# nanoporetech/scrappie

Hardware: AMD Instinct MI355X
Metric: raw samples/sec, rgrgr_r94 4k-sample reads (higher is better)
Workload: dtype f32 (3xf16 split products, 22-bit operands, fp32 accumulate)

## Files before the change

scrappie_amd/csrc/sh_eng_launch.inc:

```

struct MetaPtrs { ShMeta md; const long long *seq_off, *hp_off, *bases_off; ShGruLanes lanes, lanes1; ShGruPairs pairs, pairs2; const ShGruSegD *vseg, *vlseg; const int *vloff; ShDwellArgs dw; };

#define SH_DWELL_PER_ENTRY 10
static long long bases_reservation(long long per_entry, long long nentry) { return (per_entry * nentry + 16 + 15) & ~15ll; }
extern "C" size_t scrappie_hip_dwell_capacity(size_t nentry) { return (size_t)bases_reservation(SH_DWELL_PER_ENTRY, (long long)nentry); }

static int build_group(scrappie_hip_engine *e, Slot &sl, Model *m, const uint64_t *offsets, const uint32_t *lengths,
                       size_t n, bool hp_on, MetaPtrs &mp, const DwellJob *dw = nullptr, const PostJob *pj = nullptr) {
    LaunchGroup &lg = sl.lg;
    lg.valid = false;
    lg.n = n; lg.hp_on = hp_on;
    lg.dw = DwellJob();
    if (dw && dw->on) {
        if (m->arch != 3 || dw->off.size() != n || dw->num.size() != n || dw->host.size() != n) return set_err("build_group: %zu reads, dwells of %zu", n, dw->off.size());
        lg.dw = *dw;
    }
    lg.post = PostJob(); lg.npost = 0;
    if (pj && pj->on) {
        if (m->arch != 1 || pj->dst.size() != n) return set_err("build_group: base probabilities of %zu reads for a group of %zu (flip-flop models only)", pj->dst.size(), n);
        lg.post = *pj;
    }
    lg.ntile = (n + 15) / 16; lg.npad = lg.ntile * 16;
    const int st = m->stride;
    std::vector<int> T(n);
// ... 254 lines not shown
#ifdef SH_EXPERIMENTS
            if constexpr (nu() == 6)
                if (stamp) return launch_k<k_gru_lanes<6, true>>(lgrid, dim3(768), lds, s, xaff, out, resid, sW, sW2, md, backward, lanes, st.dev(4096 * 16 * 8));
#endif
            return launch_k<k_gru_lanes<nu(), false>>(lgrid, dim3(128 * nu()), lds, s, xaff, out, resid, sW, sW2, md, backward, lanes, (unsigned long long *)nullptr);
            })) return set_err("unsupported GRU size %d (need 32, 64 or 96 here)", S);
        if (stamp && NU == 6)
            st.dump_on(7, s, (size_t)nwg * 12 * 8, [&](const unsigned long long *h) {
                for (size_t g : {(size_t)nwg / 2}) for (int w = 0; w < 12; w++) {
                    const unsigned long long *d = &h[(g * 12 + w) * 8];
                    fprintf(stderr, "gru lanes stamp wg %zu wave %2d: phase1 %.0f bar %.0f phase2 %.0f bar %.0f cycles/step (%llu steps)\n",
                            g, w, d[0] / (double)d[4], d[1] / (double)d[4], d[2] / (double)d[4], d[3] / (double)d[4], d[4]);
                }
            });
        return rc;
    }
    if (tun().gru_debug >= 0) backward |= tun().gru_debug << 8;
    static StampBuf st1;
    unsigned long long *dbgbuf = tun().gru_stamp ? st1.dev(4096 * 8 * 8) : nullptr;
    if (dbgbuf)
        st1.dump_on(8, s, ntile * NU * 8, [&](const unsigned long long *h) {
            { unsigned long long first_end = ~0ull, mn = ~0ull, mx = 0; size_t late = 0;
              for (size_t tl = 0; tl < ntile; tl++) { first_end = std::min(first_end, h[tl * NU * 8 + 7]); mn = std::min(mn, h[tl * NU * 8 + 6]); mx = std::max(mx, h[tl * NU * 8 + 7]); }
              for (size_t tl = 0; tl < ntile; tl++) if (h[tl * NU * 8 + 6] >= first_end) late++;
              fprintf(stderr, "residency: %zu tiles, %zu started after the first one finished; span %.1f us\n", ntile, late, (mx - mn) / 100.0); }
            for (size_t tl : {size_t(0)}) for (int w = 0; w < 1; w++) {
                const unsigned long long *d = &h[(tl * NU + w) * 8];
                fprintf(stderr, "stamp tile %zu wave %d: rgemm %.0f zgemm+valu %.0f bar1 %.0f gemm2+valu %.0f bar2 %.0f (cycles/step)\n", tl, w, d[0] / (double)d[5], d[1] / (double)d[5], d[2] / (double)d[5], d[3] / (double)d[5], d[4] / (double)d[5]);
            }
        });
    if (pick_int<2, 4, 6, 8>(NU, rc, [&](auto nu) { return launch_k<k_gru<nu()>>(dim3((unsigned)ntile), dim3(64 * nu()), 0, s, xaff, out, resid, sW, sW2, md, backward, dbgbuf); })) return rc;
    return set_err("unsupported GRU size %d (need 32, 64, 96 or 128)", S);
}

#ifndef SH_FFL_NB
#define SH_FFL_NB 3
#endif
#ifndef SH_FFL_NTH
#define SH_FFL_NTH 512
#endif
static int ff_mtp(int KQ, int mtiles) {
    const size_t per_mt = ((size_t)KQ * 256 + 256) * 4;
    int mt_fit = (int)((156 * 1024) / per_mt);
    mt_fit -= mt_fit % SH_SUM_GROUP;
    return std::min(mt_fit, (mtiles + SH_SUM_GROUP - 1) / SH_SUM_GROUP * SH_SUM_GROUP);
}

template <int KQ>
static int launch_ff_lds_k(hipStream_t s, const float *in, float *E, float *sums, const unsigned *wf, const float *bf,
                           long long ncb, int mtiles, int NS, float in_div, float out_div, int ncu) {
    constexpr int NB = SH_FFL_NB, NTH = SH_FFL_NTH;
    const int mtp = ff_mtp(KQ, mtiles);
    const size_t lds = (size_t)mtp * ((size_t)KQ * 256 + 256) * 4 + 16;
    long long gx = std::min<long long>((ncb + (NTH / 64) * NB - 1) / ((NTH / 64) * NB), ncu);
    if (gx < 1) gx = 1;
    const bool dv = out_div != 1.0f;
    const bool stamp = tun().ff_stamp && !dv;
    static StampBuf st;
    unsigned long long *dbg = stamp ? st.dev(16 * 8) : nullptr;
    if (pick_bool([&](auto d) { return launch_k<k_ff_lds<KQ, NB, NTH, d()>>(dim3((unsigned)gx), dim3(NTH), lds, s, in, E, sums, wf, bf, ncb, mtiles, mtp, NS, in_div, out_div, dbg); }, dv))
        return -1;
    if (stamp)
        st.dump_on(0, s, NTH / 64 * 8, [](const unsigned long long *h) {
            for (int w = 0; w < NTH / 64; w++)
                fprintf(stderr, "ff stamp wave %d: fill %llu  B-load %llu  tiles %llu  sums %llu cycles; %llu m-tiles -> %.0f cycles per m-tile\n", w, h[w * 8], h[w * 8 + 1], h[w * 8 + 2], h[w * 8 + 3], h[w * 8 + 4], (double)h[w * 8 + 2] / (double)h[w * 8 + 4]);
        });
    return 0;
}

static int launch_ff(hipStream_t s, int S, const float *in, float *E, float *sums, const unsigned *wf, const float *bf,
                     long long ncb, int mtiles, int NS, float in_div, float out_div, int ncu) {
    int rc = 0;
    if (ncb >= 8192 && !tun().ff_reg &&
        pick_int<2, 4, 6>(S / 16, rc, [&](auto kq) { return launch_ff_lds_k<kq()>(s, in, E, sums, wf, bf, ncb, mtiles, NS, in_div, out_div, ncu); })) return rc;
    constexpr int NB = SH_FF_NB;
    const int mtp = ff_mtp(S / 16, mtiles);
    const long long gx = (ncb + 4 * NB - 1) / (4 * NB);
    dim3 grid((unsigned)std::max<long long>(gx, 1));
    if (pick_int<2, 4, 6, 8>(S / 16, rc, [&](auto kq) {
            constexpr int KQ = kq();
            return pick_bool([&](auto dv) { return launch_k<k_ff_exp<KQ, NB, dv()>>(grid, dim3(256), 0, s, in, E, sums, wf, bf, ncb, mtiles, mtp, NS, in_div, out_div); },
                             out_div != 1.0f);
        })) return rc;
    return set_err("unsupported size %d", S);
}

static bool gru_proj_ok(int K, int S) { return K == S && S % 32 == 0 && S / 16 <= 6; }

static bool conv_edge_words(const ShConvGeom &g, int N, int T, int out[4]) {
    out[0] = out[1] = out[2] = out[3] = 0;
    if (T <= 0) return true;
    unsigned irr = 0;
    bool ok = true;
    for (int t = std::max(g.c0, T - 64); t < T; t++) {
        const int kk = (t - g.c0) / g.nstepC, ii = (t - g.c0) - kk * g.nstepC;
        if (!((kk + 1) * g.nstepX <= N - g.shiftX - ii * g.st)) {
            const int j = T - 1 - t;
            if (j >= 32) ok = false; else irr |= 1u << j;
        }
    }
    const int maxCol = (N - g.shiftX) / g.nstepX;
    const int rem = (N - g.shiftX) % g.nstepX;
    const int colR = g.c0 + g.nstepC * (maxCol - 1) + rem / g.st + 1;
    const int startR = g.st - (g.padL + N - g.WL) % g.st - 1;
    out[0] = (int)irr; out[1] = colR + startR / g.st; out[2] = startR; out[3] = N;
    return ok;
}

extern "C" int scrappie_hip_conv_edge_words(int WL, int st, int F, int N, int out[4]) {
    if (WL < 1 || st < 1 || N < 1 || !out) return -1;
    return conv_edge_words(conv_geom(WL, st, F), N, (N + st - 1) / st, out) ? 1 : 0;
}

#ifdef SH_EXPERIMENTS
static int launch_gru_conv(hipStream_t s, int kst, int act, float *out, const unsigned *iW, const float *ib, const unsigned *sW,
                           const unsigned *sW2, const ShMeta &md, int backward, const ShGruLanes &lanes1, int nwg1,
                           const ShGruLanes &lanes2, int nwg2, bool two, const ShConvFuse &cf) {
    const ShGruLanes &lanes = two ? lanes2 : lanes1;
    const int nwg = two ? nwg2 : nwg1;
    if (nwg <= 0) return 0;
    HIPCHK(hipMemsetAsync(lanes.flag, 0, (size_t)lanes.ntile * 4, s));
    const size_t lds = (two ? 2 : 1) * ((size_t)4 * 3 * 2 * 64 * 4 + (size_t)2 * 3 * 6 * 256) * 4;
    dim3 grid((unsigned)nwg);
    if (tun().proj_stamp && two && kst == 3 && !act) {
        static StampBuf st;
        if (launch_k<k_gru_conv_stamp<2, 3, 0>>(grid, dim3(768), lds, s, out, iW, ib, sW, sW2, md, backward, lanes, cf, st.dev(1024 * 12 * 16))) return -1;
        st.dump_on(3, s, (size_t)nwg * 12 * 16, [&](const unsigned long long *h) {
            for (int w = 0; w < 12; w++) {
                const unsigned long long *d = &h[((size_t)(nwg / 2) * 12 + w) * 16];
                fprintf(stderr, "conv-layer stamp wave %2d (%s): A %.0f bar %.0f B %.0f bar %.0f cycles per double step (%llu steps); chunk+fetch part of B (projection) / reads+MFMA issue (recurrence) %.0f\n", w,
                        w < 6 ? "recurrence" : "projection", d[0] / (double)d[4], d[1] / (double)d[4], d[2] / (double)d[4], d[3] / (double)d[4], d[4], d[5] / (double)d[4]);
            }
        });
        return 0;
    }
    return pick_bool([&](auto t2, auto k3, auto ac) {
        return launch_k<k_gru_conv<t2() ? 2 : 1, k3() ? 3 : 5, ac() ? 1 : 0>>(grid, dim3(768), lds, s, out, iW, ib, sW, sW2, md, backward, lanes, cf);
    }, two, kst == 3, act != 0);
}
#endif
static int launch_gru_proj(hipStream_t s, int S, const float *in, float *out, const float *resid, const unsigned *iW, const float *ib,
                           const unsigned *sW, const unsigned *sW2, const ShMeta &md, int backward, const ShGruLanes &lanes1, int nwg1,
                           const ShGruLanes &lanes2, int nwg2, bool two) {
    const ShGruLanes &lanes = two ? lanes2 : lanes1;
    const int nwg = two ? nwg2 : nwg1;
    if (nwg <= 0) return 0;
    HIPCHK(hipMemsetAsync(lanes.flag, 0, (size_t)lanes.ntile * 4, s));
    const int NU = S / 16;
    size_t lds = (two ? 2 : 1) * ((size_t)4 * (NU / 2) * 2 * 64 * 4 + (size_t)2 * 3 * NU * 256) * 4;
    if (resid && SH_RESID_LDS && lds + (size_t)(two ? 2 : 1) * 3 * NU * 256 * 4 <= 160 * 1024) lds += (size_t)(two ? 2 : 1) * 3 * NU * 256 * 4;
    dim3 grid((unsigned)nwg);
    unsigned long long *const no_dbg = nullptr;
    int rc = 0;
#ifdef SH_EXPERIMENTS
    static const bool mx_on = [] { const char *v = getenv("SH_GRU_MX"); return v && atoi(v) != 0; }();
    if (mx_on && NU == 6 && two) {
        static const bool mx_stamp = getenv("SH_MX_STAMP") != nullptr;
        if (mx_stamp && !resid) {
            static StampBuf st;
            if (launch_k<k_gru_mx<false, true>>(grid, dim3(1024), lds, s, in, out, resid, iW, ib, sW, sW2, md, backward, lanes, st.dev((size_t)1024 * 16 * 10))) return -1;
            st.dump_on(7, s, (size_t)nwg * 16 * 10, [&](const unsigned long long *hb) {
                for (int w = 0; w < 16; w++) {
                    const unsigned long long *d = &hb[((size_t)(nwg / 2) * 16 + w) * 10];
                    const double n = (double)std::max<unsigned long long>(d[8], 1);
                    fprintf(stderr, "mx stamp wave %2d (%s): P1 %.0f +bar %.0f | P2 %.0f +bar %.0f | P3 %.0f +bar %.0f | P4 %.0f +bar %.0f cycles per double step (%llu steps)\n", w,
                            w < 6 ? "recurrence " : w < 12 ? "projection " : "elementwise", d[0] / n, d[1] / n, d[2] / n, d[3] / n, d[4] / n, d[5] / n, d[6] / n, d[7] / n, d[8]);
                }
            });
            return 0;
        }
        if (pick_bool([&](auto rs) { return launch_k<k_gru_mx<rs()>>(grid, dim3(1024), lds, s, in, out, resid, iW, ib, sW, sW2, md, backward, lanes, no_dbg); }, resid != nullptr))
            return -1;
        HIPCHK(hipGetLastError());
        return 0;
    }
    const bool stamp = tun().proj_stamp && NU == 6 && two && !resid;
    const bool free_run = SH_GRU_FREE_DEFAULT ? !tun().gru_barrier : tun().gru_free;
    if (free_run) {
        const size_t flds = (two ? 2 : 1) * ((size_t)4 * (NU / 2) * 2 * 64 * 4 + (size_t)3 * 3 * NU * 256) * 4 + 64;
        if (stamp) {
            static StampBuf st;
            if (launch_k<k_gru_free<6, 2, false, true>>(grid, dim3(768), flds, s, in, out, resid, iW, ib, sW, sW2, md, backward, lanes, st.dev(1024 * 12 * 16))) return -1;
            st.dump_on(7, s, (size_t)nwg * 12 * 16, [&](const unsigned long long *h) {
                for (int w = 0; w < 12; w++) {
                    const unsigned long long *d = &h[((size_t)(nwg / 2) * 12 + w) * 16];
                    if (w < 6) fprintf(stderr, "free stamp wave %2d (recurrence): work %.0f, waiting for gate inputs %.0f, for r*h of all waves %.0f, for h of all waves %.0f cycles per double step (%llu steps)\n",
                                       w, d[0] / (double)d[4], d[1] / (double)d[4], d[2] / (double)d[4], d[3] / (double)d[4], d[4]);
                    else fprintf(stderr, "free stamp wave %2d (projection): work %.0f, waiting for the column's pieces %.0f, for a free ring slot %.0f cycles per double step (%llu steps)\n",
                                 w, d[0] / (double)d[4], d[1] / (double)d[4], d[2] / (double)d[4], d[4]);
                }
            });
            return 0;
        }
        if (pick_int<2, 4, 6>(NU, rc, [&](auto nu) {
                constexpr int N = nu();
                return pick_bool([&](auto t2, auto rs) {
                    return launch_k<k_gru_free<N, t2() ? 2 : 1, rs(), false>>(grid, dim3(128 * N), flds, s, in, out, resid, iW, ib, sW, sW2, md, backward, lanes, no_dbg);
                }, two, resid != nullptr);
            })) return rc;
        return set_err("unsupported GRU size %d (need 32, 64 or 96 here)", S);
    }
    if (stamp) {
        static StampBuf st;
        if (launch_k<k_gru_proj<6, 2, false, true>>(grid, dim3(768), lds, s, in, out, resid, iW, ib, sW, sW2, md, backward, lanes, st.dev(1024 * 12 * 16))) return -1;
        st.dump_on(7, s, (size_t)nwg * 12 * 16, [&](const unsigned long long *h) {
            for (int w = 0; w < 12; w++) {
                const unsigned long long *d = &h[((size_t)(nwg / 2) * 12 + w) * 16];
                fprintf(stderr, "proj stamp wave %2d (%s): A %.0f bar %.0f B %.0f bar %.0f cycles per double step (%llu steps)", w, w < 6 ? "recurrence" : "projection",
                        d[0] / (double)d[4], d[1] / (double)d[4], d[2] / (double)d[4], d[3] / (double)d[4], d[4]);
                if (w < 6) fprintf(stderr, "; inside B: reads+MFMA issue %.0f, logistic z %.0f, tanh+blend %.0f, store+bookkeeping %.0f, cut+publish %.0f",
                                   d[5] / (double)d[4], d[6] / (double)d[4], d[7] / (double)d[4], d[8] / (double)d[4], d[9] / (double)d[4]);
                fprintf(stderr, "\n");
            }
        });
        return 0;
    }
#endif
    if (pick_int<2, 4, 6>(NU, rc, [&](auto nu) {
            constexpr int N = nu();
            return pick_bool([&](auto t2) {
                constexpr int NT = t2() ? 2 : 1;
                if (resid) return launch_k<k_gru_proj_res<N, NT>>(grid, dim3(128 * N), lds, s, in, out, resid, iW, ib, sW, sW2, md, backward, lanes);
                return launch_k<k_gru_proj<N, NT, false>>(grid, dim3(128 * N), lds, s, in, out, resid, iW, ib, sW, sW2, md, backward, lanes, no_dbg);
            }, two);
        })) return rc;
    return set_err("unsupported GRU size %d (need 32, 64 or 96 here)", S);
}

#ifdef SH_EXPERIMENTS
#ifndef SH_GRU32_DEFAULT
#define SH_GRU32_DEFAULT 0
#endif
static int use_gru32(const scrappie_hip_engine *e) {
    if (e->dbg_gru32 >= 0) return e->dbg_gru32;
    if (SH_GRU32_DEFAULT ? tun().gru16 : !tun().gru32) return 0;
    const char *v = getenv("SH_GRU32");
    return (v && atoi(v) == 2) ? 2 : (SH_GRU32_DEFAULT ? SH_GRU32_DEFAULT : 1);
}
static const char *const g32_role[8] = {"R0 chain", "R1 chain", "R2 chain", "C cand-proj", "G0 z/r", "G1 z/r", "G2 z/r", "L loader"};
static int launch_gru_proj32x2(hipStream_t s, const float *in, float *out, bool resid, const unsigned *iW, const float *ib, const unsigned *sW,
                               const unsigned *sW2, const ShMeta &md, int backward, const ShGruPairs &pairs, int nwg, size_t ntile) {
    if (nwg <= 0) return 0;
    HIPCHK(hipMemsetAsync(pairs.flag, 0, ntile * 4, s));
    const size_t lds = (size_t)SH_G32X2_LDS_WORDS * 4;
    dim3 grid((unsigned)nwg);
    if (tun().gru32_stamp && !resid) {
        static StampBuf st;
        if (launch_k<k_gru_proj32x2<false, true>>(grid, dim3(512), lds, s, in, out, iW, ib, sW, sW2, md, backward, pairs, st.dev(1024 * 8 * 16))) return -1;
        st.dump_on(7, s, (size_t)nwg * 8 * 16, [&](const unsigned long long *h) {
            for (int w = 0; w < 8; w++) {
                const unsigned long long *d = &h[((size_t)(nwg / 2) * 8 + w) * 16];
                fprintf(stderr, "gru32x2 stamp wave %d (%s): work %.0f bar %.0f cycles per interval (%llu intervals = one tile-step of 32 reads each)\n", w, g32_role[w],
                        d[0] / (double)d[4], d[1] / (double)d[4], d[4]);
            }
        });
        return 0;
    }
    return pick_bool([&](auto rs) { return launch_k<k_gru_proj32x2<rs(), false>>(grid, dim3(512), lds, s, in, out, iW, ib, sW, sW2, md, backward, pairs, (unsigned long long *)nullptr); }, resid);
}
static int launch_gru_proj32(hipStream_t s, const float *in, float *out, bool resid, const unsigned *iW, const float *ib, const unsigned *sW,
                             const unsigned *sW2, const ShMeta &md, int backward, const ShGruPairs &pairs, int nwg, size_t ntile) {
    if (nwg <= 0) return 0;
    HIPCHK(hipMemsetAsync(pairs.flag, 0, ntile * 4, s));
    const size_t lds = (size_t)SH_G32_LDS_WORDS * 4;
    dim3 grid((unsigned)nwg);
    if (tun().gru32_stamp && !resid) {
        static StampBuf st;
        if (launch_k<k_gru_proj32<false, true>>(grid, dim3(512), lds, s, in, out, iW, ib, sW, sW2, md, backward, pairs, st.dev(1024 * 8 * 16))) return -1;
        st.dump_on(7, s, (size_t)nwg * 8 * 16, [&](const unsigned long long *h) {
            for (int w = 0; w < 8; w++) {
                const unsigned long long *d = &h[((size_t)(nwg / 2) * 8 + w) * 16];
                fprintf(stderr, "gru32 stamp wave %d (%s): A %.0f bar %.0f B %.0f bar %.0f cycles per step (%llu steps)", w, g32_role[w],
                        d[0] / (double)d[4], d[1] / (double)d[4], d[2] / (double)d[4], d[3] / (double)d[4], d[4]);
                if (w < 3) fprintf(stderr, "; A: reads+r products %.0f, logistic*h %.0f, cut+write %.0f; B: reads+candidate products %.0f, z/tanh/blend %.0f, store %.0f, cut+write %.0f",
                                   d[5] / (double)d[4], d[6] / (double)d[4], d[7] / (double)d[4], d[8] / (double)d[4], d[9] / (double)d[4], d[10] / (double)d[4], d[11] / (double)d[4]);
                fprintf(stderr, "\n");
            }
        });
        return 0;
    }
    return pick_bool([&](auto rs) { return launch_k<k_gru_proj32<rs(), false>>(grid, dim3(512), lds, s, in, out, iW, ib, sW, sW2, md, backward, pairs, (unsigned long long *)nullptr); }, resid);
}

#endif
static int launch_lstm(hipStream_t s, int S, const float *xaff, float *out, const unsigned *sW, const float *pf,
                       const ShMeta &md, int backward, const ShGruLanes &lanes, int nwg) {
    if (nwg <= 0) return 0;
    HIPCHK(hipMemsetAsync(lanes.flag, 0, (size_t)lanes.ntile * 4, s));
    int rc = 0;
    if (pick_int<2, 4, 6>(S / 16, rc, [&](auto nu) { return launch_k<k_lstm_lanes<nu()>>(dim3((unsigned)nwg), dim3(128 * nu()), 0, s, xaff, out, sW, pf, md, backward, lanes); })) return rc;
    return set_err("unsupported LSTM size %d (need 32, 64 or 96)", S);
}

static int launch_lstm_proj(hipStream_t s, int S, int I, const float *in, float *out, const unsigned *iW, const float *ib,
                            const unsigned *sW, const float *pf, const ShMeta &md, int backward, const ShGruLanes &lanes, int nwg) {
    if (nwg <= 0) return 0;
    HIPCHK(hipMemsetAsync(lanes.flag, 0, (size_t)lanes.ntile * 4, s));
    const int NU = S / 16;
    const size_t lds = ((size_t)4 * (NU / 2) * 2 * 64 * 4 + (size_t)2 * 4 * NU * 256 + (size_t)3 * NU * 256) * 4;
    if (I != S && I != 16) return set_err("unsupported LSTM input width %d", I);
    int rc = 0;
    if (pick_int<2, 4, 6>(NU, rc, [&](auto nu) {
            constexpr int N = nu();
            return pick_bool([&](auto wide) { return launch_k<k_lstm_proj<N, wide() ? N : 1>>(dim3((unsigned)nwg), dim3(128 * N), lds, s, in, out, iW, ib, sW, pf, md, backward, lanes); },
                             I == S);
        })) return rc;
    return set_err("unsupported LSTM size %d (need 32, 64 or 96)", S);
}

static size_t viterbi_lds_bytes(int NH) {
    const int nskip = NH / 16, nslip = std::max(NH / 64, 1);
    return (size_t)NH * 16 * 4 * 2 + (size_t)nskip * 16 * 8 + (size_t)nslip * 16 * 8 + 2 * 16 * 16 * 8;
}

static int launch_viterbi(hipStream_t s, int NH, const ShVitArgs &a, const ShMeta &md, size_t nwg) {
    const size_t lds = viterbi_lds_bytes(NH);
    if (nwg == 0) return 0;
    const bool fin = a.sums != nullptr, slip = a.use_slip != 0, skip0 = a.skip_pen == 0.0f;
    if (fin && !a.want_log) return set_err("decode: exp-value input implies log output");
    const auto go = [&](auto nth, auto ppt) {
        constexpr int NTH = nth(), PPT = ppt();
        return pick_bool([&](auto fi, auto sl, auto sk) { return launch_k<k_viterbi<NTH, PPT, fi(), sl(), sk()>>(dim3((unsigned)nwg), dim3(NTH), lds, s, a, md); },
                         fin, slip, skip0);
    };
    switch (NH) {
    case 64: return go(int_c<256>(), int_c<1>());
    case 256: return go(int_c<256>(), int_c<4>());
    case 1024:
#ifdef SH_EXPERIMENTS
        if (getenv("SH_VIT_1024")) return go(int_c<1024>(), int_c<4>());
#endif
        return go(int_c<512>(), int_c<8>());
    default: return set_err("unsupported transducer state count %d (need 4^3, 4^4 or 4^5 k-mers)", NH);
    }
}

static int launch_ff_viterbi(hipStream_t s, const ShFfArgs &f, const ShVitArgs &a, const ShMeta &md, size_t nwg, bool single) {
    const size_t lds = (size_t)SH_FV_LDS_FLOATS * 4;
    if (nwg == 0) return 0;
    dim3 grid((unsigned)nwg);
    const bool slip = a.use_slip != 0, skip0 = a.skip_pen == 0.0f, dv = f.out_div != 1.0f || f.in_div != 1.0f;
    if (!a.use_slip && !single) {
        const size_t ldt = (size_t)SH_FVT_LDS_FLOATS * 4;
        static const bool keep_clamp = getenv("SH_FVT_KEEP_CLAMP") != nullptr;
        const bool nc = f.no_clamp && !dv && !keep_clamp;
        return pick_bool([&](auto sk, auto d, auto n) {
            if constexpr (d() && n()) return -1;
            else return launch_k<k_ff_viterbi_teams<sk(), d(), n()>>(grid, dim3(SH_FVT_NTH), ldt, s, f, a, md);
        }, skip0, dv, nc);
    }
    return pick_bool([&](auto sl, auto sk, auto d) { return launch_k<k_ff_viterbi<sl(), sk(), d()>>(grid, dim3(512), lds, s, f, a, md); }, slip, skip0, dv);
}
```

scrappie_amd/csrc/sh_gru.h:

```cpp
#ifndef SH_GRU_H
#define SH_GRU_H

template <int NU>
__global__ __launch_bounds__(64 * NU) void k_gru(const float *__restrict__ xaff, float *__restrict__ out,
                                                 const float *__restrict__ resid,
                                                 const float *__restrict__ sWfrag ,
                                                 const float *__restrict__ sW2frag ,
                                                 ShMeta md, int backward, unsigned long long *dbgbuf) {
    constexpr int KR = NU * 4;
    const int dbg = backward >> 8;
    backward &= 1;
    __shared__ __attribute__((aligned(16))) float lds[2 * NU * 256];
    float *lds_h = lds, *lds_rh = lds + NU * 256;
    const int lane = threadIdx.x & 63, u = threadIdx.x >> 6;
    const int tile = blockIdx.x;
    const int Tt = md.tile_T[tile];
    const long long boff = md.tile_boff[tile];
    const int myT = md.rT[tile * 16 + (lane & 15)];

    float wz[KR], wr[KR], wh[KR];
#pragma unroll
    for (int r = 0; r < KR; r++) {
        wz[r] = sWfrag[((long long)u * KR + r) * 64 + lane];
        wr[r] = sWfrag[((long long)(NU + u) * KR + r) * 64 + lane];
// ... 325 lines not shown
    auto fetch_next = [&](int i) {
        n_ok = i < sge;
        if (n_ok) {
            const ShGruSegD sg = L.seg[i];
            n_tile = __builtin_amdgcn_readfirstlane(sg.tile);
            n_s0 = __builtin_amdgcn_readfirstlane(sg.s0);
            n_s1 = __builtin_amdgcn_readfirstlane(sg.s1);
            n_Tt = __builtin_amdgcn_readfirstlane(md.tile_T[n_tile]);
            n_boff = __builtin_amdgcn_readfirstlane((int)md.tile_boff[n_tile]);
            n_myT = md.rT[n_tile * 16 + (lane & 15)];
        }
    };
    auto advance = [&]() { tile = n_tile; s = n_s0; s1 = n_s1; Tt = n_Tt; boff = n_boff; myT = n_myT; };
    f32x4 h = {0.f, 0.f, 0.f, 0.f};
    auto take_over = [&]() {
        h = (f32x4){0.f, 0.f, 0.f, 0.f};
        if (s > 0) {
            if (!sh_wait_flag(L.flag + tile, (unsigned)NU, L.flag + L.ntile) && lane == 0)
                __hip_atomic_store(L.flag + L.ntile, 1u, __ATOMIC_RELAXED, __HIP_MEMORY_SCOPE_AGENT);
            __builtin_amdgcn_fence(__ATOMIC_ACQUIRE, "agent");
            const float *hs = L.hstate + ((long long)tile * NU + u) * 256 + lane * 4;
#pragma unroll
            for (int k = 0; k < 4; k++) h[k] = __hip_atomic_load(hs + k, __ATOMIC_RELAXED, __HIP_MEMORY_SCOPE_AGENT);
        }
    };
    f32x4 xz = h, xr = h, xh = h;
    auto xload = [&](long long col) {
        const float *p = xaff + col * xstride + lane * 4;
        xz = *(const f32x4 *)(p + u * 256);
        xr = *(const f32x4 *)(p + (NU + u) * 256);
        xh = *(const f32x4 *)(p + (2 * NU + u) * 256);
    };
    if (my_it > 0) {
        fetch_next(sgi);
        advance();
        fetch_next(++sgi);
        take_over();
        publish(lds_h, h);
        xload(boff + (backward ? Tt - 1 - s : s));
    }
    __syncthreads();

    int it = 0;
    for (; it < my_it; it++) {
        f32x4 ar = xr * SH_OSCALE, az = xz * SH_OSCALE, ah = xh * SH_OSCALE;
        const int t = backward ? Tt - 1 - s : s;
        {
            long long ncol = boff + t;
            if (s + 1 < s1) ncol = boff + (backward ? t - 1 : t + 1);
            else if (n_ok) ncol = n_boff + (backward ? n_Tt - 1 - n_s0 : n_s0);
            xload(ncol);
        }
        {
            ShSplit hp[KS];
#pragma unroll
            for (int ks = 0; ks < KS; ks++) hp[ks] = pieces(lds_h, ks);
            split_dot2<KS>(wr, wz, hp, ar, az);
        }
        publish(lds_rh, d_logistic4_acc(ar) * h);
        const f32x4 z = d_logistic4_acc(az);
        lds_barrier();
        {
            ShSplit rp[KS];
#pragma unroll
            for (int ks = 0; ks < KS; ks++) rp[ks] = pieces(lds_rh, ks);
            ah = split_dot<KS>(wh, rp, ah);
        }
        const bool active = t < myT;
        {
            const f32x4 hbar = d_tanh4_acc(ah);
            const f32x4 hn = z * h + (1.0f - z) * hbar;
#pragma unroll
            for (int k = 0; k < 4; k++) h[k] = active ? hn[k] : 0.0f;
        }
        f32x4 o = h;
        const long long oidx = ((long long)(boff + t) * NU + u) * 256 + lane * 4;
        if (resid) o += *(const f32x4 *)(resid + oidx);
        *(f32x4 *)(out + oidx) = o;
        s++;
        if (s == s1) {
            if (s1 < Tt) {
                float *hs = L.hstate + ((long long)tile * NU + u) * 256 + lane * 4;
#pragma unroll
                for (int k = 0; k < 4; k++) __hip_atomic_store(hs + k, h[k], __ATOMIC_RELAXED, __HIP_MEMORY_SCOPE_AGENT);
                __builtin_amdgcn_fence(__ATOMIC_RELEASE, "agent");
                if (lane == 0) __hip_atomic_fetch_add(L.flag + tile, 1u, __ATOMIC_RELEASE, __HIP_MEMORY_SCOPE_AGENT);
            }
            if (n_ok) {
                advance();
                fetch_next(++sgi);
                take_over();
            }
        }
        publish(lds_h, h);
        lds_barrier();
    }
    for (; it < nit; it++) { lds_barrier(); lds_barrier(); }
}

struct ShLaneCursor {
    int sgi, sge;
    int tile, s, s1, Tt, boff;
    bool ok;
};

#ifndef SH_REC45_PRIO
#define SH_REC45_PRIO 0
#endif
#ifndef SH_REC_PRIO
#define SH_REC_PRIO 0
#endif
#ifndef SH_PDELAY_A
#define SH_PDELAY_A 0
#endif
#ifndef SH_PDELAY_B
#define SH_PDELAY_B 0
#endif
#ifndef SH_PROJ_PRIO
#define SH_PROJ_PRIO 0
#endif
#ifndef SH_RFIRST
#define SH_RFIRST 1
#endif
#ifndef SH_PROJ_VALU_FIRST
#define SH_PROJ_VALU_FIRST 1
#endif
#ifndef SH_PROJ_INPLACE
#define SH_PROJ_INPLACE 1
#endif
#ifndef SH_ABL
#define SH_ABL 0
#endif
__device__ __forceinline__ f32x4 abl_logistic4(f32x4 a) { return (SH_ABL & 1) ? a * (0.25f * SH_OINV) + 0.5f : d_logistic4_acc(a); }
__device__ __forceinline__ f32x4 abl_tanh4(f32x4 a) { return (SH_ABL & 1) ? a * (0.5f * SH_OINV) : d_tanh4_acc(a); }

#ifndef SH_GRU_VGPR_HALF
#define SH_GRU_VGPR_HALF 72
#endif
#ifndef SH_FUSE_ABL
#define SH_FUSE_ABL 0
#endif
struct ShConvFuse {
    const float *sig;
    const float *W;
    const float *bias;
    const int *edge;
    unsigned *bad;
    ShConvGeom g;
};

#ifndef SH_RESID_LDS
#define SH_RESID_LDS 1
#endif
template <int NU, int NT, bool RESID, bool STAMP, int KST, int ACT>
__device__ __forceinline__ void gru_proj_body(const float *__restrict__ in, float *__restrict__ out,
                                              const float *__restrict__ resid,
                                              const unsigned *__restrict__ iWp, const float *__restrict__ ibfrag,
                                              const unsigned *__restrict__ sWp, const unsigned *__restrict__ sW2p,
                                              const ShMeta &md, int backward, const ShGruLanes &L,
                                              unsigned long long *dbg, const ShConvFuse &cf) {
    constexpr bool CONV = KST > 0;
    static_assert(NU % 2 == 0, "k steps of 32 units");
    constexpr int KS = NU / 2;
    constexpr int PBUF = KS * 2 * 64 * 4;
    constexpr int XBUF = 3 * NU * 256;
    constexpr int TBUF = 4 * PBUF + 2 * XBUF;
    constexpr int RBUF = NU * 256;
    constexpr bool RLDS = RESID && !CONV && SH_RESID_LDS && (NT * (TBUF + 3 * RBUF) * 4 <= 160 * 1024);
    unsigned long long pa = 0, pb = 0, pc = 0, pd = 0, pt0 = 0, pt1;
    unsigned long long q1 = 0, q2 = 0, q3 = 0, q4 = 0, q5 = 0, qt0 = 0, qt1;
#define QSTAMP(acc) do { if (STAMP) { qt1 = __builtin_readcyclecounter(); acc += qt1 - qt0; qt0 = qt1; } } while (0)
#define PSTAMP(acc) do { if (STAMP) { pt1 = __builtin_readcyclecounter(); acc += pt1 - pt0; pt0 = pt1; } } while (0)
#define PDUMP() do { if (STAMP && dbg && lane == 0) { unsigned long long *d_ = dbg + ((long long)blockIdx.x * 2 * NU + wave) * 16; d_[0] = pa; d_[1] = pb; d_[2] = pc; d_[3] = pd; d_[4] = nit; d_[5] = q1; d_[6] = q2; d_[7] = q3; d_[8] = q4; d_[9] = q5; } } while (0)
    extern __shared__ __attribute__((aligned(16))) unsigned ldsw[];
    const int lane = threadIdx.x & 63;
    const unsigned lofs = (unsigned)lane * 4u;
    typedef __attribute__((address_space(1))) float *gf32;
    typedef __attribute__((address_space(1))) f32x4 *gf32x4;
    auto gload = [&](const float *base) { gf32 b = (gf32)base; asm volatile("" : "+s"(b)); return *(gf32x4)(b + lofs); };
    auto gstore = [&](float *base, f32x4 v) { gf32 b = (gf32)base; asm volatile("" : "+s"(b)); *(gf32x4)(b + lofs) = v; };
    const int wave = __builtin_amdgcn_readfirstlane(threadIdx.x >> 6);
    const bool rec = wave < NU;
    const int u = rec ? wave : wave - NU;

    ShSplit w0[KS], w1[KS], w2[KS];
    {
        const unsigned *f0 = rec ? sWp + (long long)u * KS * 512 : iWp + (long long)u * KS * 512;
        const unsigned *f1 = rec ? sWp + (long long)(NU + u) * KS * 512 : iWp + (long long)(NU + u) * KS * 512;
        const unsigned *f2 = rec ? sW2p + (long long)u * KS * 512 : iWp + (long long)(2 * NU + u) * KS * 512;
#pragma unroll
        for (int ks = 0; ks < KS; ks++) {
            w0[ks] = load_pieces(f0 + ks * 512, lane);
            w1[ks] = load_pieces(f1 + ks * 512, lane);
            w2[ks] = load_pieces(f2 + ks * 512, lane);
        }
#pragma unroll
        for (int ks = 0; ks < KS; ks++)
            asm volatile("" : "+v"(w0[ks].p1), "+v"(w0[ks].p2), "+v"(w1[ks].p1), "+v"(w1[ks].p2), "+v"(w2[ks].p1), "+v"(w2[ks].p2));
    }
    const int wofs = (((u >> 1) * 2) * 64 + lane) * 4 + (u & 1) * 2;
    auto publish = [&](unsigned *buf, f32x4 v) {
        unsigned a1, a2, b1, b2;
        if (SH_ABL & 4) { a1 = __float_as_uint(v[0]); a2 = __float_as_uint(v[1]); b1 = __float_as_uint(v[2]); b2 = __float_as_uint(v[3]); }
        else { split_pair(v[0], v[1], a1, a2); split_pair(v[2], v[3], b1, b2); }
        *(uint2 *)(buf + wofs) = make_uint2(a1, b1);
        *(uint2 *)(buf + wofs + 256) = make_uint2(a2, b2);
    };
    auto pieces = [&](const unsigned *buf, int ks) { return load_pieces(buf + ks * 512, lane); };
    auto lds_h = [&](int tl) { return ldsw + tl * TBUF; };
    auto lds_rh = [&](int tl) { return ldsw + tl * TBUF + PBUF; };
    auto lds_in = [&](int tl, int par) { return ldsw + tl * TBUF + (2 + par) * PBUF; };
    auto lds_x = [&](int tl, int par) { return (float *)(ldsw + tl * TBUF + 4 * PBUF + par * XBUF); };
    auto lds_raw = [&](int tl, int slot) { return (float *)(ldsw + NT * TBUF + (tl * 3 + slot) * RBUF) + (u * 64 + lane) * 4; };

    ShLaneCursor c[NT] = {};
    int my_it[NT], nit = 0;
#pragma unroll
    for (int tl = 0; tl < NT; tl++) {
        const int ln = blockIdx.x * NT + tl;
        c[tl].sgi = __builtin_amdgcn_readfirstlane(L.lane_off[ln]);
        c[tl].sge = __builtin_amdgcn_readfirstlane(L.lane_off[ln + 1]);
        int n = 0;
        for (int i = c[tl].sgi; i < c[tl].sge; i++) n += L.seg[i].s1 - L.seg[i].s0;
        my_it[tl] = __builtin_amdgcn_readfirstlane(n);
        nit = max(nit, my_it[tl]);
    }
    if (nit == 0) return;
    auto enter = [&](ShLaneCursor &cc) {
        cc.ok = cc.sgi < cc.sge;
        if (cc.ok) {
            const ShGruSegD sg = L.seg[cc.sgi];
            cc.tile = __builtin_amdgcn_readfirstlane(sg.tile);
            cc.s = __builtin_amdgcn_readfirstlane(sg.s0);
            cc.s1 = __builtin_amdgcn_readfirstlane(sg.s1);
            cc.Tt = __builtin_amdgcn_readfirstlane(md.tile_T[cc.tile]);
            cc.boff = __builtin_amdgcn_readfirstlane((int)md.tile_boff[cc.tile]);
        }
    };
    auto column = [&](const ShLaneCursor &cc) { return (long long)cc.boff + (backward ? cc.Tt - 1 - cc.s : cc.s); };

    if (!rec) {
        if (SH_PROJ_PRIO) __builtin_amdgcn_s_setprio(SH_PROJ_PRIO);
        f32x4 bz = *(const f32x4 *)(ibfrag + (u * 64 + lane) * 4);
        f32x4 br = *(const f32x4 *)(ibfrag + ((NU + u) * 64 + lane) * 4);
        asm volatile("" : "+v"(bz), "+v"(br));
        f32x4 bh = *(const f32x4 *)(ibfrag + ((2 * NU + u) * 64 + lane) * 4);
        asm volatile("" : "+v"(bh));
        int e_irr[NT], e_pw[NT], e_N[NT], e_T[NT];
        unsigned e_soff[NT];
        float ca[CONV ? KST : 1];
        f32x4 cb = {0.f, 0.f, 0.f, 0.f};
        auto read_consts = [&](int tl) {
            if (CONV && c[tl].ok) {
                const int rd = c[tl].tile * 16 + (lane & 15);
                const int4 ev = ((const int4 *)cf.edge)[rd];
                e_irr[tl] = ev.x; e_pw[tl] = ev.y * 16 + ev.z; e_N[tl] = ev.w;
                e_T[tl] = md.rT[rd];
                e_soff[tl] = (unsigned)md.sig_off[rd];
            }
        };
        if (CONV) {
#pragma unroll
            for (int ks = 0; ks < (CONV ? KST : 1); ks++)
                ca[ks] = (4 * ks + (lane >> 4) < cf.g.WL) ? cf.W[(4 * ks + (lane >> 4)) * cf.g.F + 16 * u + (lane & 15)] : 0.0f;
            cb = *(const f32x4 *)(cf.bias + 16 * u + 4 * (lane >> 4));
#pragma unroll
            for (int tl = 0; tl < NT; tl++) { e_irr[tl] = 0; e_pw[tl] = 0; e_N[tl] = 0; e_T[tl] = 0; e_soff[tl] = 0u; }
        }
        struct XQ { f32x4 v; float xs[CONV ? KST : 1]; int meta; int tile; };
        auto fetch = [&](ShLaneCursor &cc, int tl) {
            XQ x;
            x.meta = 0; x.tile = 0;
            if constexpr (!CONV) {
                const long long col = cc.ok ? column(cc) : 0;
                x.v = gload(in + (col * NU + u) * 256);
            } else {
                const int tb = cc.ok ? (backward ? cc.Tt - 1 - cc.s : cc.s) : 0;
                const bool live = cc.ok && tb < e_T[tl];
                const int j = e_T[tl] - 1 - tb;
                const bool regular = live && !(j < 32 && ((e_irr[tl] >> (j & 31)) & 1));
                const int base = tb * cf.g.st - cf.g.padL + (lane >> 4);
                typedef __attribute__((address_space(1))) float *gsf;
                gsf sb = (gsf)cf.sig; asm volatile("" : "+s"(sb));
                int okbits = 0;
#pragma unroll
                for (int ks = 0; ks < KST; ks++) {
                    const int idx = base + 4 * ks;
                    const bool ok = regular && 4 * ks + (lane >> 4) < cf.g.WL && idx >= 0 && idx < e_N[tl];
                    x.xs[ks] = (SH_FUSE_ABL & 1) ? (float)idx : *(sb + (e_soff[tl] + (unsigned)(ok ? idx : 0)));
                    okbits |= ok ? (256 << ks) : 0;
                }
                const int jw = tb - (e_pw[tl] >> 4);
                const int wp = (e_pw[tl] & 15) + jw * cf.g.st;
                x.meta = (live ? ((jw >= 0 && wp < cf.g.padR) ? wp + 2 : 1) : 0) | okbits;
                x.tile = cc.tile;
            }
            if (cc.ok) {
                cc.s++;
                if (cc.s == cc.s1) { cc.sgi++; enter(cc); read_consts(tl); }
            }
            return x;
        };
        auto chunk_of = [&](const XQ &x) {
            if constexpr (!CONV) return x.v;
            else {
                f32x4 acc = cb;
#pragma unroll
                for (int ks = 0; ks < KST; ks++) { if (SH_FUSE_ABL & 2) acc[0] += ca[ks] * x.xs[ks]; else acc = mfma4(ca[ks], ((x.meta >> (8 + ks)) & 1) ? x.xs[ks] : 0.0f, acc); }
                const int rd = x.tile * 16 + (lane & 15);
                const int colcode = x.meta & 255;
                if (!(SH_FUSE_ABL & 4) && colcode >= 2) {
                    const int N = md.rN[rd], w = colcode - 2;
                    const float *xp = cf.sig + md.sig_off[rd] + (N - cf.g.WL + 1 + w);
                    const int f0 = 16 * u + 4 * (lane >> 4);
                    for (int tap = 0; tap < cf.g.WL - w - 1; tap++) {
                        const f32x4 wv = *(const f32x4 *)(cf.W + tap * cf.g.F + f0);
                        acc += wv * xp[tap];
                    }
                }
                if (colcode == 0) acc = f32x4{0.f, 0.f, 0.f, 0.f};
                else if (!(SH_FUSE_ABL & 8)) {
                    bool out_of_range = false;
#pragma unroll
                    for (int r = 0; r < 4; r++) {
                        const float v = ACT ? d_tanh(acc[r]) : d_elu(acc[r]);
                        out_of_range |= !(__builtin_fabsf(v) < SH_ACT_LIMIT) | !(__builtin_fabsf(acc[r]) <= 3.0e38f);
                        acc[r] = (v == v) ? __builtin_amdgcn_fmed3f(v, -SH_ACT_LIMIT, SH_ACT_LIMIT) : 0.0f;
                    }
                    if (out_of_range && cf.bad) cf.bad[rd] = 1u;
                }
                return acc;
            }
        };
        XQ xq1[NT], xq2[NT];
        auto project_h = [&](const unsigned *ibuf, float *xdst) {
            ShSplit ip[KS];
#pragma unroll
            for (int ks = 0; ks < KS; ks++) ip[ks] = pieces(ibuf, ks);
            const f32x4 dst = (SH_ABL & 8) ? bh : split_dot<KS>(w2, ip, bh);
            *(f32x4 *)(xdst + ((2 * NU + u) * 64 + lane) * 4) = dst;
            if ((SH_ABL & 16) && !(u == 2 || u == 3)) {
                const f32x4 extra = split_dot<KS>(w0, ip, bh);
                asm volatile("" :: "v"(extra));
            }
        };
        auto project_zr = [&](const unsigned *ibuf, float *xdst) {
            f32x4 cz = bz, cr = br;
            if (!(SH_ABL & 8) && !((SH_ABL & 16) && (u == 2 || u == 3))) {
                ShSplit ip[KS];
#pragma unroll
                for (int ks = 0; ks < KS; ks++) ip[ks] = pieces(ibuf, ks);
                split_dot2<KS>(w0, w1, ip, cz, cr);
            }
            *(f32x4 *)(xdst + (u * 64 + lane) * 4) = cz;
            *(f32x4 *)(xdst + ((NU + u) * 64 + lane) * 4) = cr;
        };
#pragma unroll
        for (int tl = 0; tl < NT; tl++) {
            enter(c[tl]);
            read_consts(tl);
            const XQ xin = fetch(c[tl], tl);
            xq1[tl] = fetch(c[tl], tl); xq2[tl] = fetch(c[tl], tl);
            publish(lds_in(tl, 0), chunk_of(xin));
            if constexpr (RLDS) *(f32x4 *)lds_raw(tl, 0) = chunk_of(xin);
        }
        lds_barrier();
#pragma unroll
        for (int tl = 0; tl < NT; tl++) {
            project_h(lds_in(tl, 0), lds_x(tl, 0));
            project_zr(lds_in(tl, 0), lds_x(tl, 0));
            publish(lds_in(tl, 1), chunk_of(xq1[tl]));
            if constexpr (RLDS) *(f32x4 *)lds_raw(tl, 1) = chunk_of(xq1[tl]);
            xq1[tl] = xq2[tl];
            xq2[tl] = fetch(c[tl], tl);
        }
        lds_barrier();
        if (STAMP) pt0 = __builtin_readcyclecounter();
        int wslot = 2;
        if constexpr (CONV || SH_PROJ_INPLACE) {
            auto step = [&](int it, const int par, XQ (&e)[NT]) {
                const int np = par ^ 1;
#pragma unroll
                for (int tl = 0; tl < NT; tl++) project_h(lds_in(tl, np), lds_x(tl, np));
                PSTAMP(pa);
                lds_barrier();
                PSTAMP(pb);
#pragma unroll
                for (int tl = 0; tl < NT; tl++) {
                    publish(lds_in(tl, par), chunk_of(e[tl]));
                    if constexpr (RLDS) *(f32x4 *)lds_raw(tl, wslot) = chunk_of(e[tl]);
                    e[tl] = fetch(c[tl], tl);
                }
                if constexpr (RLDS) wslot = wslot == 2 ? 0 : wslot + 1;
                __builtin_amdgcn_sched_barrier(0);
                if (STAMP) { qt1 = __builtin_readcyclecounter(); q1 += qt1 - pt0; }
#pragma unroll
                for (int tl = 0; tl < NT; tl++) project_zr(lds_in(tl, np), lds_x(tl, np));
                PSTAMP(pc);
                lds_barrier();
                PSTAMP(pd);
            };
            for (int it = 0; it < nit; it += 2) {
                step(it, 0, xq1);
                if (it + 1 < nit) step(it + 1, 1, xq2);
            }
        } else
        for (int it = 0; it < nit; it++) {
            const int np = (it + 1) & 1;
            if (SH_PDELAY_A) __builtin_amdgcn_s_sleep(SH_PDELAY_A);
#pragma unroll
            for (int tl = 0; tl < NT; tl++) project_h(lds_in(tl, np), lds_x(tl, np));
            PSTAMP(pa);
            lds_barrier();
            PSTAMP(pb);
            if (SH_PROJ_VALU_FIRST) {
#pragma unroll
                for (int tl = 0; tl < NT; tl++) {
                    publish(lds_in(tl, it & 1), chunk_of(xq1[tl]));
                    if constexpr (RLDS) *(f32x4 *)lds_raw(tl, wslot) = chunk_of(xq1[tl]);
                    xq1[tl] = xq2[tl];
                    xq2[tl] = fetch(c[tl], tl);
                }
                __builtin_amdgcn_sched_barrier(0);
            }
            if (SH_PDELAY_B) __builtin_amdgcn_s_sleep(SH_PDELAY_B);
#pragma unroll
            for (int tl = 0; tl < NT; tl++) project_zr(lds_in(tl, np), lds_x(tl, np));
            if (!SH_PROJ_VALU_FIRST) {
#pragma unroll
                for (int tl = 0; tl < NT; tl++) {
                    publish(lds_in(tl, it & 1), chunk_of(xq1[tl]));
                    if constexpr (RLDS) *(f32x4 *)lds_raw(tl, wslot) = chunk_of(xq1[tl]);
                    xq1[tl] = xq2[tl];
                    xq2[tl] = fetch(c[tl], tl);
                }
            }
            if constexpr (RLDS) wslot = wslot == 2 ? 0 : wslot + 1;
            PSTAMP(pc);
            lds_barrier();
            PSTAMP(pd);
        }
        PDUMP();
        return;
    }

    if (SH_REC_PRIO) __builtin_amdgcn_s_setprio(SH_REC_PRIO);
    if (SH_REC45_PRIO && NU == 6 && wave >= 4) __builtin_amdgcn_s_setprio(SH_REC45_PRIO);
    static_assert(NT <= 2, "two block counts per register");
    unsigned myT2 = 0;
    f32x4 h[NT];
    auto take_over = [&](int tl) {
        h[tl] = (f32x4){0.f, 0.f, 0.f, 0.f};
        int mt = 0;
        if (c[tl].ok) mt = md.rT[c[tl].tile * 16 + (lane & 15)];
        if (NT == 1) myT2 = (unsigned)mt;
        else myT2 = tl ? ((myT2 & 0xffffu) | ((unsigned)mt << 16)) : ((myT2 & 0xffff0000u) | ((unsigned)mt & 0xffffu));
        if (!c[tl].ok) return;
        if (c[tl].s > 0) {
            if (!sh_wait_flag(L.flag + c[tl].tile, (unsigned)NU, L.flag + L.ntile) && lane == 0)
                __hip_atomic_store(L.flag + L.ntile, 1u, __ATOMIC_RELAXED, __HIP_MEMORY_SCOPE_AGENT);
            __builtin_amdgcn_fence(__ATOMIC_ACQUIRE, "agent");
            const float *hs = L.hstate + ((long long)c[tl].tile * NU + u) * 256 + lane * 4;
#pragma unroll
            for (int k = 0; k < 4; k++) h[tl][k] = __hip_atomic_load(hs + k, __ATOMIC_RELAXED, __HIP_MEMORY_SCOPE_AGENT);
        }
        asm volatile("" : "+v"(myT2), "+v"(h[tl][0]), "+v"(h[tl][1]), "+v"(h[tl][2]), "+v"(h[tl][3]));
    };
    long long oix[NT];
    const long long dstep = backward ? -(long long)(NU * 256) : (long long)(NU * 256);
    auto cur_off = [&](int tl) {
        const long long v = c[tl].ok ? (column(c[tl]) * NU + u) * 256 : (long long)(u * 256);
        const unsigned lo = __builtin_amdgcn_readfirstlane((unsigned)v), hi = __builtin_amdgcn_readfirstlane((unsigned)(v >> 32));
        return (long long)(((unsigned long long)hi << 32) | lo);
    };
#pragma unroll
    for (int tl = 0; tl < NT; tl++) {
        enter(c[tl]);
        take_over(tl);
        oix[tl] = cur_off(tl);
        publish(lds_h(tl), h[tl]);
    }
    lds_barrier();
    lds_barrier();
    if (STAMP) pt0 = __builtin_readcyclecounter();
    f32x4 rs[NT];
    auto resid_fetch = [&](int tl) {
        rs[tl] = gload(resid + oix[tl]);
    };
    if (RESID && !RLDS) {
#pragma unroll
        for (int tl = 0; tl < NT; tl++) resid_fetch(tl);
    }
    int rslot = 0;
    for (int it = 0; it < nit; it++) {
        const int par = it & 1;
        f32x4 cr[NT], cz[NT];
        f32x4 z[NT];
        if (SH_RFIRST) {
            ShSplit hp[NT][KS];
#pragma unroll
            for (int tl = 0; tl < NT; tl++) {
                const float *xs = lds_x(tl, par);
                cz[tl] = *(const f32x4 *)(xs + (u * 64 + lane) * 4);
                cr[tl] = *(const f32x4 *)(xs + ((NU + u) * 64 + lane) * 4);
#pragma unroll
                for (int ks = 0; ks < KS; ks++) hp[tl][ks] = pieces(lds_h(tl), ks);
                cr[tl] = split_dot<KS>(w1, hp[tl], cr[tl]);
            }
#pragma unroll
            for (int tl = 0; tl < NT; tl++) cz[tl] = split_dot<KS>(w0, hp[tl], cz[tl]);
#pragma unroll
            for (int tl = 0; tl < NT; tl++) publish(lds_rh(tl), abl_logistic4(cr[tl]) * h[tl]);
        } else {
#pragma unroll
        for (int tl = 0; tl < NT; tl++) {
            const float *xs = lds_x(tl, par);
            cz[tl] = *(const f32x4 *)(xs + (u * 64 + lane) * 4);
            cr[tl] = *(const f32x4 *)(xs + ((NU + u) * 64 + lane) * 4);
            ShSplit hp[KS];
#pragma unroll
            for (int ks = 0; ks < KS; ks++) hp[ks] = pieces(lds_h(tl), ks);
            split_dot2<KS>(w1, w0, hp, cr[tl], cz[tl]);
        }
#pragma unroll
        for (int tl = 0; tl < NT; tl++) {
            publish(lds_rh(tl), abl_logistic4(cr[tl]) * h[tl]);
            z[tl] = abl_logistic4(cz[tl]);
        }
        }
        PSTAMP(pa);
        lds_barrier();
        PSTAMP(pb);
        if (STAMP) qt0 = __builtin_readcyclecounter();
        f32x4 ch[NT];
#pragma unroll
        for (int tl = 0; tl < NT; tl++) {
            ShSplit rp[KS];
#pragma unroll
            for (int ks = 0; ks < KS; ks++) rp[ks] = pieces(lds_rh(tl), ks);
            ch[tl] = split_dot<KS>(w2, rp, *(const f32x4 *)(lds_x(tl, par) + ((2 * NU + u) * 64 + lane) * 4));
            if (STAMP) __builtin_amdgcn_sched_barrier(0);
            QSTAMP(q1);
        }
        if (SH_RFIRST) {
#pragma unroll
            for (int tl = 0; tl < NT; tl++) z[tl] = abl_logistic4(cz[tl]);
        }
        if (STAMP) { asm volatile("" :: "v"(z[0]), "v"(z[NT - 1])); __builtin_amdgcn_sched_barrier(0); }
        QSTAMP(q2);
#pragma unroll
        for (int tl = 0; tl < NT; tl++) {
            const bool live = it < my_it[tl];
            const int t = backward ? c[tl].Tt - 1 - c[tl].s : c[tl].s;
            const bool active = t < (int)(NT == 1 ? myT2 : (tl ? (myT2 >> 16) : (myT2 & 0xffffu)));
            if constexpr (RLDS) rs[tl] = *(const f32x4 *)lds_raw(tl, rslot);
            {
                const f32x4 hbar = abl_tanh4(ch[tl]);
                const f32x4 hn = z[tl] * h[tl] + (1.0f - z[tl]) * hbar;
#pragma unroll
                for (int k = 0; k < 4; k++) h[tl][k] = active ? hn[k] : 0.0f;
            }
            if (STAMP) { asm volatile("" :: "v"(h[tl])); __builtin_amdgcn_sched_barrier(0); }
            QSTAMP(q3);
            if (live) {
// ... 83 lines not shown
```

Measured before the change: 1.682 billion.

## Shift projection m-tiles off busiest waves into the h-interval of other waves

For the NU=6, two-tile, non-residual GRU projection kernel, the r-gate (and optionally z-gate) m-tile work of waves 2 and 3 is moved to other waves. Those waves stage the extra weight pieces and bias in added LDS and compute them alongside their h projection in the first interval. The goal is to balance MFMA work between the two barrier-separated intervals, so that waves 2 and 3 stop being the critical path. The cost is extra LDS per workgroup and LDS weight reads, which could lower occupancy. The partial-product ordering inside the split dot also changes.

New measurement: 1.680 billion. Within noise of the previous version (-0.1%).

```diff
diff --git a/scrappie_amd/csrc/sh_eng_launch.inc b/scrappie_amd/csrc/sh_eng_launch.inc
--- a/scrappie_amd/csrc/sh_eng_launch.inc
+++ b/scrappie_amd/csrc/sh_eng_launch.inc
@@ -430,6 +430,7 @@
     dim3 grid((unsigned)nwg);
     unsigned long long *const no_dbg = nullptr;
     int rc = 0;
+    const size_t plds = lds + (sh_proj_shift_on(NU, two ? 2 : 1, resid != nullptr, false) ? (size_t)SH_PROJ_SHIFT_WORDS * 4 : 0);
 #ifdef SH_EXPERIMENTS
     static const bool mx_on = [] { const char *v = getenv("SH_GRU_MX"); return v && atoi(v) != 0; }();
     if (mx_on && NU == 6 && two) {
@@ -480,7 +481,7 @@
     }
     if (stamp) {
         static StampBuf st;
-        if (launch_k<k_gru_proj<6, 2, false, true>>(grid, dim3(768), lds, s, in, out, resid, iW, ib, sW, sW2, md, backward, lanes, st.dev(1024 * 12 * 16))) return -1;
+        if (launch_k<k_gru_proj<6, 2, false, true>>(grid, dim3(768), plds, s, in, out, resid, iW, ib, sW, sW2, md, backward, lanes, st.dev(1024 * 12 * 16))) return -1;
         st.dump_on(7, s, (size_t)nwg * 12 * 16, [&](const unsigned long long *h) {
             for (int w = 0; w < 12; w++) {
                 const unsigned long long *d = &h[((size_t)(nwg / 2) * 12 + w) * 16];
@@ -499,7 +500,7 @@
             return pick_bool([&](auto t2) {
                 constexpr int NT = t2() ? 2 : 1;
                 if (resid) return launch_k<k_gru_proj_res<N, NT>>(grid, dim3(128 * N), lds, s, in, out, resid, iW, ib, sW, sW2, md, backward, lanes);
-                return launch_k<k_gru_proj<N, NT, false>>(grid, dim3(128 * N), lds, s, in, out, resid, iW, ib, sW, sW2, md, backward, lanes, no_dbg);
+                return launch_k<k_gru_proj<N, NT, false>>(grid, dim3(128 * N), plds, s, in, out, resid, iW, ib, sW, sW2, md, backward, lanes, no_dbg);
             }, two);
         })) return rc;
     return set_err("unsupported GRU size %d (need 32, 64 or 96 here)", S);
diff --git a/scrappie_amd/csrc/sh_gru.h b/scrappie_amd/csrc/sh_gru.h
--- a/scrappie_amd/csrc/sh_gru.h
+++ b/scrappie_amd/csrc/sh_gru.h
@@ -501,6 +501,13 @@
 #ifndef SH_RESID_LDS
 #define SH_RESID_LDS 1
 #endif
+#ifndef SH_PROJ_SHIFT
+#define SH_PROJ_SHIFT 2
+#endif
+static_assert(SH_PROJ_SHIFT == 0 || SH_PROJ_SHIFT == 2 || SH_PROJ_SHIFT == 4, "m-tiles moved off waves 8, 9");
+constexpr bool sh_proj_shift_on(int NU, int NT, bool resid, bool conv) { return SH_PROJ_SHIFT != 0 && NU == 6 && NT == 2 && !resid && !conv; }
+constexpr int SH_PROJ_SHIFT_MT_WORDS = 3 * 512;
+constexpr int SH_PROJ_SHIFT_WORDS = SH_PROJ_SHIFT * (SH_PROJ_SHIFT_MT_WORDS + 256);
 template <int NU, int NT, bool RESID, bool STAMP, int KST, int ACT>
 __device__ __forceinline__ void gru_proj_body(const float *__restrict__ in, float *__restrict__ out,
                                               const float *__restrict__ resid,
@@ -595,6 +602,22 @@
         asm volatile("" : "+v"(bz), "+v"(br));
         f32x4 bh = *(const f32x4 *)(ibfrag + ((2 * NU + u) * 64 + lane) * 4);
         asm volatile("" : "+v"(bh));
+        constexpr bool SHIFT = sh_proj_shift_on(NU, NT, RESID, CONV);
+        const bool gave_r = SHIFT && (u == 2 || u == 3), gave_z = gave_r && SH_PROJ_SHIFT == 4;
+        const int xk = !SHIFT ? -1 : SH_PROJ_SHIFT == 4 ? (u < 2 ? u : u >= 4 ? u - 2 : -1) : (u < 2 ? u : -1);
+        const int xmt = SH_PROJ_SHIFT == 4 ? (xk & 1) * NU + 2 + (xk >> 1) : NU + 2 + xk;
+        unsigned *const xa = ldsw + NT * TBUF + (xk < 0 ? 0 : xk) * (SH_PROJ_SHIFT_MT_WORDS + 256);
+        float *const xb = (float *)(xa + SH_PROJ_SHIFT_MT_WORDS) + lane * 4;
+        if (SHIFT && xk >= 0) {
+            *(f32x4 *)xb = *(const f32x4 *)(ibfrag + (xmt * 64 + lane) * 4);
+#pragma unroll
+            for (int ks = 0; ks < KS; ks++) {
+                const ShSplit a = load_pieces(iWp + ((long long)xmt * KS + ks) * 512, lane);
+                *(u32x4 *)(xa + ks * 512 + lane * 4) = __builtin_bit_cast(u32x4, a.p1);
+                *(u32x4 *)(xa + ks * 512 + 256 + lane * 4) = __builtin_bit_cast(u32x4, a.p2);
+            }
+        }
+        auto xpiece = [&](int ks, int p) { return __builtin_bit_cast(f16x8, *(const u32x4 *)(xa + ks * 512 + p * 256 + lane * 4)); };
         int e_irr[NT], e_pw[NT], e_N[NT], e_T[NT];
         unsigned e_soff[NT];
         float ca[CONV ? KST : 1];
@@ -682,27 +705,85 @@
             }
         };
         XQ xq1[NT], xq2[NT];
+        auto fresh = [&](const void *p) { unsigned o = (unsigned)((const unsigned *)p - ldsw); asm volatile("" : "+s"(o)); return ldsw + o; };
         auto project_h = [&](const unsigned *ibuf, float *xdst) {
+            if constexpr (SHIFT) { ibuf = fresh(ibuf); xdst = (float *)fresh(xdst); }
             ShSplit ip[KS];
 #pragma unroll
             for (int ks = 0; ks < KS; ks++) ip[ks] = pieces(ibuf, ks);
             const f32x4 dst = (SH_ABL & 8) ? bh : split_dot<KS>(w2, ip, bh);
             *(f32x4 *)(xdst + ((2 * NU + u) * 64 + lane) * 4) = dst;
-            if ((SH_ABL & 16) && !(u == 2 || u == 3)) {
-                const f32x4 extra = split_dot<KS>(w0, ip, bh);
-                asm volatile("" :: "v"(extra));
-            }
+        };
+        auto project_h_shift = [&](const unsigned *ibuf_, float *xdst_) {
+            const unsigned *ibuf = fresh(ibuf_);
+            float *xdst = (float *)fresh(xdst_);
+            f32x4 ch = bh, cx = *(const f32x4 *)xb;
+            auto ipiece = [&](int ks, int p) { return __builtin_bit_cast(f16x8, *(const u32x4 *)(ibuf + ks * 512 + p * 256 + lane * 4)); };
+#pragma unroll
+            for (int ks = 0; ks < KS; ks++) {
+                const f16x8 b2 = ipiece(ks, 1), a1 = xpiece(ks, 0);
+                ch = mfma16(w2[ks].p1, b2, ch); cx = mfma16(a1, b2, cx);
+            }
+            f16x8 b1[KS];
+#pragma unroll
+            for (int ks = 0; ks < KS; ks++) {
+                b1[ks] = ipiece(ks, 0);
+                const f16x8 a2 = xpiece(ks, 1);
+                ch = mfma16(w2[ks].p2, b1[ks], ch); cx = mfma16(a2, b1[ks], cx);
+            }
+            asm volatile("" ::: "memory");
+#pragma unroll
+            for (int ks = 0; ks < KS; ks++) {
+                const f16x8 a1 = xpiece(ks, 0);
+                ch = mfma16(w2[ks].p1, b1[ks], ch); cx = mfma16(a1, b1[ks], cx);
+            }
+            *(f32x4 *)(xdst + ((2 * NU + u) * 64 + lane) * 4) = ch;
+            *(f32x4 *)(xdst + (xmt * 64 + lane) * 4) = cx;
         };
         auto project_zr = [&](const unsigned *ibuf, float *xdst) {
+            if (gave_z) return;
             f32x4 cz = bz, cr = br;
-            if (!(SH_ABL & 8) && !((SH_ABL & 16) && (u == 2 || u == 3))) {
+            if (SHIFT && !(SH_ABL & 8)) {
+                ibuf = fresh(ibuf); xdst = (float *)fresh(xdst);
+                f16x8 b[KS];
+#pragma unroll
+                for (int ks = 0; ks < KS; ks++) b[ks] = __builtin_bit_cast(f16x8, *(const u32x4 *)(ibuf + ks * 512 + 256 + lane * 4));
+                if (gave_r) {
+#pragma unroll
+                    for (int ks = 0; ks < KS; ks++) cz = mfma16(w0[ks].p1, b[ks], cz);
+                } else {
+#pragma unroll
+                    for (int ks = 0; ks < KS; ks++) { cz = mfma16(w0[ks].p1, b[ks], cz); cr = mfma16(w1[ks].p1, b[ks], cr); }
+                }
+                __builtin_amdgcn_sched_barrier(0);
+#pragma unroll
+                for (int ks = 0; ks < KS; ks++) b[ks] = __builtin_bit_cast(f16x8, *(const u32x4 *)(ibuf + ks * 512 + lane * 4));
+                if (gave_r) {
+#pragma unroll
+                    for (int ks = 0; ks < KS; ks++) cz = mfma16(w0[ks].p2, b[ks], cz);
+#pragma unroll
+                    for (int ks = 0; ks < KS; ks++) cz = mfma16(w0[ks].p1, b[ks], cz);
+                } else {
+#pragma unroll
+                    for (int ks = 0; ks < KS; ks++) { cz = mfma16(w0[ks].p2, b[ks], cz); cr = mfma16(w1[ks].p2, b[ks], cr); }
+#pragma unroll
+                    for (int ks = 0; ks < KS; ks++) { cz = mfma16(w0[ks].p1, b[ks], cz); cr = mfma16(w1[ks].p1, b[ks], cr); }
+                }
+            } else if (!(SH_ABL & 8)) {
                 ShSplit ip[KS];
 #pragma unroll
                 for (int ks = 0; ks < KS; ks++) ip[ks] = pieces(ibuf, ks);
                 split_dot2<KS>(w0, w1, ip, cz, cr);
             }
             *(f32x4 *)(xdst + (u * 64 + lane) * 4) = cz;
-            *(f32x4 *)(xdst + ((NU + u) * 64 + lane) * 4) = cr;
+            if (!gave_r) *(f32x4 *)(xdst + ((NU + u) * 64 + lane) * 4) = cr;
+        };
+        auto interval_a = [&](int np) {
+#pragma unroll
+            for (int tl = 0; tl < NT; tl++) {
+                if (SHIFT && xk >= 0) project_h_shift(lds_in(tl, np), lds_x(tl, np));
+                else project_h(lds_in(tl, np), lds_x(tl, np));
+            }
         };
 #pragma unroll
         for (int tl = 0; tl < NT; tl++) {
@@ -714,9 +795,9 @@
             if constexpr (RLDS) *(f32x4 *)lds_raw(tl, 0) = chunk_of(xin);
         }
         lds_barrier();
+        interval_a(0);
 #pragma unroll
         for (int tl = 0; tl < NT; tl++) {
-            project_h(lds_in(tl, 0), lds_x(tl, 0));
             project_zr(lds_in(tl, 0), lds_x(tl, 0));
             publish(lds_in(tl, 1), chunk_of(xq1[tl]));
             if constexpr (RLDS) *(f32x4 *)lds_raw(tl, 1) = chunk_of(xq1[tl]);
@@ -729,8 +810,7 @@
         if constexpr (CONV || SH_PROJ_INPLACE) {
             auto step = [&](int it, const int par, XQ (&e)[NT]) {
                 const int np = par ^ 1;
-#pragma unroll
-                for (int tl = 0; tl < NT; tl++) project_h(lds_in(tl, np), lds_x(tl, np));
+                interval_a(np);
                 PSTAMP(pa);
                 lds_barrier();
                 PSTAMP(pb);
@@ -757,8 +837,7 @@
         for (int it = 0; it < nit; it++) {
             const int np = (it + 1) & 1;
             if (SH_PDELAY_A) __builtin_amdgcn_s_sleep(SH_PDELAY_A);
-#pragma unroll
-            for (int tl = 0; tl < NT; tl++) project_h(lds_in(tl, np), lds_x(tl, np));
+            interval_a(np);
             PSTAMP(pa);
             lds_barrier();
             PSTAMP(pb);
```
